# tjcunhao/dpo

Measured on NVIDIA H100. Metric: rtr_iters_per_sec_sphere2500, higher is better.
Workload: dtype f64

## Files before the change

### dpo_b200/csrc/dpgo_kernels.cu

```cuda
#include "dpgo_device.cuh"
#include "dpgo_kernels.cuh"
#include "dpgo_rotation.cuh"
#include <cooperative_groups.h>
#include <algorithm>

namespace dpgo {

struct BlockCtx {
  double *sm_warp;
  double *sm_out;
  unsigned epoch;
  int parity;
};

template <int NUSED = NRED>
__device__ __forceinline__ void phase_end(const KParams &kp, BlockCtx &bc, double (&acc)[NRED]) {
  const int lane = threadIdx.x & 31, warp = threadIdx.x >> 5, nwarps = blockDim.x >> 5;
#pragma unroll
  for (int q = 0; q < NUSED; ++q) {
    double v = warp_sum(acc[q]);
    if (lane == 0) bc.sm_warp[warp * NRED + q] = v;
  }
  __syncthreads();
  bc.epoch += gridDim.x;
  double *slot = kp.partials + (size_t)bc.parity * kp.grid * NRED;
  double *outp = bc.sm_out + bc.parity * NRED;
  if (warp == 0) {
    if (NUSED > 0) {
      double s[NUSED > 0 ? NUSED : 1];
#pragma unroll
      for (int q = 0; q < NUSED; ++q) {
        double v = (lane < nwarps) ? bc.sm_warp[lane * NRED + q] : 0.0;
        s[q] = warp_sum(v);
      }
      if (lane == 0) {
#pragma unroll
        for (int q = 0; q < NUSED; ++q) slot[(size_t)blockIdx.x * NRED + q] = s[q];
      }
    }
    if (!kp.cluster) {
      if (lane == 0) asm volatile("red.release.gpu.global.add.u32 [%0], 1;" ::"l"(kp.bar_counter) : "memory");
      if (kp.strict_acquire) { while ((int)(ld_acquire_u32(kp.bar_counter) - bc.epoch) < 0) { } }
      else { while ((int)(ld_relaxed_u32(kp.bar_counter) - bc.epoch) < 0) { } }
    }
  }
  if (kp.cluster) {
    asm volatile("barrier.cluster.arrive.release.aligned;" ::: "memory");
    if (kp.strict_acquire) asm volatile("barrier.cluster.wait.acquire.aligned;" ::: "memory");
    else asm volatile("barrier.cluster.wait.aligned;" ::: "memory");
  }
  if (warp == 0) {
    if (NUSED > 0) {
      double t[NUSED > 0 ? NUSED : 1];
#pragma unroll
      for (int q = 0; q < NUSED; ++q) t[q] = 0.0;
      for (int c = lane; c < kp.grid; c += 32) {
#pragma unroll
        for (int q = 0; q < NUSED; ++q) t[q] += __ldcg(slot + (size_t)c * NRED + q);
      }
#pragma unroll
      for (int q = 0; q < NUSED; ++q) {
        const double v = warp_sum(t[q]);
        if (lane == 0) outp[q] = v;
      }
    }
  }
  __syncthreads();
#pragma unroll
  for (int q = 0; q < NUSED; ++q) acc[q] = outp[q];
  bc.parity ^= 1;
}

struct CtaRows {
  int r0, r1;
  const int *rowptr;
  const int *bcol;
  const double *bval;
};

template <int R> struct RowIter {
  static constexpr int SG = SubGroup<R>::SG;
  int r0, r1, stride, jb, sgw, a, c;
  __device__ RowIter(const CtaRows &cr) {
    r0 = cr.r0;
    r1 = cr.r1;
    const int lane = threadIdx.x & 31;
    constexpr int SGW = 32 / SG;
    sgw = lane / SG;
    stride = (blockDim.x >> 5) * SGW;
    jb = r0 + (threadIdx.x >> 5) * SGW;
    const int l = lane & (SG - 1);
    a = l >> 2;
    c = l & 3;
  }
};

template <int R, int DH>
__device__ void phase_eval(const KParams &kp, const CtaRows &cr, int cb, bool save_xin, int precond, double (&acc)[NRED]) {
  constexpr int TS = R * DH;
  const double *X = kp.v[V_X0 + cb];
  double *EG = kp.v[V_EG0 + cb], *RG = kp.v[V_RG0 + cb], *Z0 = kp.v[V_Z00 + cb], *S = kp.S[cb];
  RowIter<R> it(cr);
  const bool valid = (it.a < R) && (it.c < DH);
  const int e = it.c * R + it.a;
  for (int jb = it.jb; jb < it.r1; jb += it.stride) {
    const int j = jb + it.sgw;
    const bool act = (j < it.r1);
    const int js = act ? j : it.r1 - 1;
    const bool ld = act && valid;
    double xq = gather_tile<R, DH, true, false>(cr.rowptr, cr.bcol, cr.bval, X, nullptr, 0.0, js, it.a, it.c);
    const size_t idx = (size_t)js * TS + e;
    const double x = ld ? __ldcg(X + idx) : 0.0;
    const double g = ld ? __ldcg(kp.G + idx) : 0.0;
    if (!ld) xq = 0.0;
    const double eg = xq + g;
    acc[0] = fma(xq, x, acc[0]);
    acc[1] = fma(x, g, acc[1]);
    double ya[3], sym[3];
    const double rg = tangent_project_elem<R, DH>(x, eg, it.a, it.c, ya, sym);
    if (ld) {
      EG[idx] = eg;
      RG[idx] = rg;
      if (save_xin) kp.v[V_XIN][idx] = x;
      acc[2] = fma(rg, rg, acc[2]);
    }
    if (act && it.a == 0 && it.c < 3) {
      double *s = S + (size_t)js * 9 + it.c * 3;
      s[0] = sym[0]; s[1] = sym[1]; s[2] = sym[2];
    }
    if (precond != DPGO_PRECOND_DENSE_EXACT && precond != DPGO_PRECOND_SPARSE_EXACT) {
      double z0 = rg;
      if (precond == DPGO_PRECOND_BLOCK_JACOBI) {
        double t = jacobi_elem<R, DH>(kp.dinv, js, ld ? rg : 0.0, it.a, it.c);
        double ya2[3], sym2[3];
        z0 = tangent_project_elem<R, DH>(x, t, it.a, it.c, ya2, sym2);
      }
      if (ld) {
        Z0[idx] = z0;
        acc[3] = fma(z0, rg, acc[3]);
      }
    }
  }
}

template <int R, int DH, bool CLOCK>
__device__ void phase_hess(const KParams &kp, const CtaRows &cr, int cb, const double *zsrc, const double *dold, double *dnew,
                           double beta, bool onfly, double (&acc)[NRED]) {
  constexpr int TS = R * DH;
  constexpr int D = DH - 1;
  const double *X = kp.v[V_X0 + cb];
  const double *S = kp.S[cb];
  double *HD = kp.v[V_HD];
  RowIter<R> it(cr);
  const bool valid = (it.a < R) && (it.c < DH);
  const int e = it.c * R + it.a;
  const bool ticking = CLOCK && (kp.phase_ns != nullptr) && blockIdx.x == 0 && threadIdx.x == 0;
  unsigned long long th0 = 0, th1 = 0;
  if (ticking) asm volatile("mov.u64 %0, %%globaltimer;" : "=l"(th0));
  for (int jb = it.jb; jb < it.r1; jb += it.stride) {
    const int j = jb + it.sgw;
    const bool act = (j < it.r1);
    const int js = act ? j : it.r1 - 1;
    const bool ld = act && valid;
    const size_t idx = (size_t)js * TS + e;
    double dl = 0.0, dprev = 0.0;
    if (ld) {
      dl = __ldcg(zsrc + idx);
      if (onfly && beta != 0.0) dprev = __ldcg(dold + idx);
    }
    const double x = ld ? __ldcg(X + idx) : 0.0;
    const bool rot = ld && (it.c < D);
    double s0 = 0, s1 = 0, s2 = 0;
    if (rot) {
      const double *s = S + (size_t)js * 9 + it.c * 3;
      s0 = __ldcg(s); s1 = __ldcg(s + 1); s2 = __ldcg(s + 2);
    }
    double hq;
    if (onfly) hq = gather_tile<R, DH, true, true>(cr.rowptr, cr.bcol, cr.bval, zsrc, dold, beta, js, it.a, it.c);
    else hq = gather_tile<R, DH, true, false>(cr.rowptr, cr.bcol, cr.bval, zsrc, nullptr, 0.0, js, it.a, it.c);
    if (ticking && jb == it.jb) { asm volatile("mov.u64 %0, %%globaltimer;" : "=l"(th1)); kp.phase_ns[27] += th1 - th0; }
    if (ld && onfly) {
      dl = -dl;
      if (beta != 0.0) dl = fma(beta, dprev, dl);
      dnew[idx] = dl;
    }
    const double dr = rot ? dl : 0.0;
    const double d0 = quad_get(dr, 0), d1 = quad_get(dr, 1), d2 = (D > 2) ? quad_get(dr, 2) : 0.0;
    double w = ld ? hq : 0.0;
    if (rot) w -= (d0 * s0 + d1 * s1 + d2 * s2);
    double ya[3], sym[3];
    const double hd = tangent_project_elem<R, DH>(x, w, it.a, it.c, ya, sym);
    if (ld) {
      HD[idx] = hd;
      acc[0] = fma(dl, hd, acc[0]);
    }
  }
  if (ticking) { asm volatile("mov.u64 %0, %%globaltimer;" : "=l"(th1)); kp.phase_ns[28] += th1 - th0; }
}

template <int R, int DH>
__device__ void phase_update(const KParams &kp, const CtaRows &cr, int cb, const double *dcur, double alpha, bool first, int precond,
                             double (&acc)[NRED]) {
  constexpr int TS = R * DH;
  const double *X = kp.v[V_X0 + cb];
  const double *RG = kp.v[V_RG0 + cb];
  double *ETA = kp.v[V_ETA], *RES = kp.v[V_RES], *Z = kp.v[V_Z];
  const double *HD = kp.v[V_HD];
  RowIter<R> it(cr);
  const bool valid = (it.a < R) && (it.c < DH);
  const int e = it.c * R + it.a;
  for (int jb = it.jb; jb < it.r1; jb += it.stride) {
    const int j = jb + it.sgw;
    const bool act = (j < it.r1);
    const int js = act ? j : it.r1 - 1;
    const bool ld = act && valid;
    const size_t idx = (size_t)js * TS + e;
    double res = 0.0, x = 0.0;
    if (ld) {
      const double dl = __ldcg(dcur + idx), hd = __ldcg(HD + idx);
      const double eta0 = first ? 0.0 : __ldcg(ETA + idx);
      const double res0 = first ? __ldcg(RG + idx) : __ldcg(RES + idx);
      res = fma(alpha, hd, res0);
      ETA[idx] = fma(alpha, dl, eta0);
      RES[idx] = res;
// ... 520 lines not shown
          }
        }
        d0 += f0;
        d1 += f1;
        {
          double *sl = slots + (size_t)slot * SLOT + r8 * R + 2 * k4;
          if (2 * k4 < R) sl[0] = accum ? sl[0] + d0 : d0;
          if (2 * k4 + 1 < R) sl[1] = accum ? sl[1] + d1 : d1;
        }
        ji = jn; ja = na; jb = nb;
      }
    }
    __syncthreads();
    if (ticking) asm volatile("mov.u64 %0, %%globaltimer;" : "=l"(tg2));
    {
      int eb = e0 + warp * SGW;
      int4 ea = make_int4(-1, 0, 0, 0), ec = make_int4(0, 0, 0, 0), ed = make_int4(0, 0, 0, 0);
      if (eb + sgw < e1) {
        const int4 *rp = reinterpret_cast<const int4 *>(N.epis + eb + sgw);
        ea = __ldg(rp); ec = __ldg(rp + 1); ed = __ldg(rp + 2);
      }
      while (eb < e1) {
        const int en = eb + nsub;
        int4 fa = make_int4(-1, 0, 0, 0), fc = make_int4(0, 0, 0, 0), fd = make_int4(0, 0, 0, 0);
        if (en + sgw < e1) {
          const int4 *rp = reinterpret_cast<const int4 *>(N.epis + en + sgw);
          fa = __ldg(rp); fc = __ldg(rp + 1); fd = __ldg(rp + 2);
        }
        const bool act = (eb + sgw < e1);
        const int kind = ea.x, slot0 = ea.y, nslots = ea.z, half = ea.w, out = ec.x, aux = ec.y, nc = ec.z, cext = ec.w;
        const bool ld = act && valid;
        const bool sol = (kind == nd::EPI_ROOT) || (kind == nd::EPI_B_OWN);
        double tval = 0.0, xq = 0.0, vv = 0.0, cv[NC] = {0.0, 0.0, 0.0, 0.0};
        if (ld) {
          if (kind == nd::EPI_B_OWN) tval = __ldcg(N.TX + (size_t)out * TS + e);
          if (sol) { xq = __ldcg(X + (size_t)aux * TS + e); vv = __ldcg(V + (size_t)aux * TS + e); }
          if (kind == nd::EPI_F_BND) {
            const int ci[NC] = {ed.x, ed.y, ed.z, ed.w};
#pragma unroll
            for (int q = 0; q < NC; ++q) cv[q] = (q < nc) ? __ldcg(N.C + (size_t)ci[q] * TS + e) : 0.0;
          }
        }
        double sum = 0.0;
        if (ld) {
          const double *sl = slots + (size_t)slot0 * SLOT + (half * DH + c) * R + a;
          for (int k = 0; k < nslots; ++k) sum += sl[(size_t)k * SLOT];
        }
        double x = 0.0;
        if (ld) {
          if (kind == nd::EPI_F_OWN) {
            N.TX[(size_t)out * TS + e] = sum;
          } else if (kind == nd::EPI_F_BND) {
#pragma unroll
            for (int q = 0; q < NC; ++q) sum += cv[q];
            for (int k = NC; k < nc; ++k) sum += __ldcg(N.C + (size_t)ld_const(N.csrc + cext + k - NC) * TS + e);
            N.C[(size_t)out * TS + e] = sum;
          } else if (sol) {
            x = (kind == nd::EPI_ROOT) ? sum : tval - sum;
            N.TX[(size_t)out * TS + e] = x;
          }
        }
        if (__any_sync(FULL, sol)) {
          double ya[3], sym[3];
          const double z = tangent_project_elem<R, DH>(sol ? xq : 0.0, x, a, c, ya, sym);
          if (ld && sol) {
            Zout[(size_t)aux * TS + e] = z;
            acc[0] = fma(z, vv, acc[0]);
          }
        }
        eb = en; ea = fa; ec = fc; ed = fd;
      }
    }
    if (ticking) {
      unsigned long long tg3;
      asm volatile("mov.u64 %0, %%globaltimer;" : "=l"(tg3));
      kp.phase_ns[24] += tg1 - tg0; kp.phase_ns[25] += tg2 - tg1; kp.phase_ns[26] += tg3 - tg2;
      unsigned long long *pp = kp.phase_ns + 32 + 3 * min(ph, 9);
      pp[0] += tg1 - tg0; pp[1] += tg2 - tg1; pp[2] += tg3 - tg2;
    }
    if (si + 1 < s1) __syncthreads();
  }
}

template <int R, int DH>
__device__ void phase_retract(const KParams &kp, const CtaRows &cr, int cb, int mode, const double *dcur, double tau, bool eta_zero,
                              double step, double (&acc)[NRED]) {
  constexpr int TS = R * DH;
  const double *X = kp.v[V_X0 + cb];
  const double *RG = kp.v[V_RG0 + cb];
  double *X2 = kp.v[V_X0 + (1 - cb)];
  RowIter<R> it(cr);
  const bool valid = (it.a < R) && (it.c < DH);
  const int e = it.c * R + it.a;
  for (int jb = it.jb; jb < it.r1; jb += it.stride) {
    const int j = jb + it.sgw;
    const bool act = (j < it.r1);
    const int js = act ? j : it.r1 - 1;
    const bool ld = act && valid;
    const size_t idx = (size_t)js * TS + e;
    double w = 0.0;
    if (ld) {
      const double x = __ldcg(X + idx);
      double eta;
      if (mode == 1) {
        eta = -step * __ldcg(RG + idx);
      } else if (mode == 2) {
        eta = __ldcg(kp.v[V_AUX] + idx);
      } else {
        const double g = __ldcg(RG + idx);
        eta = eta_zero ? 0.0 : __ldcg(kp.v[V_ETA] + idx);
        double heta = eta_zero ? 0.0 : (__ldcg(kp.v[V_RES] + idx) - g);
        if (tau != 0.0) {
          eta = fma(tau, __ldcg(dcur + idx), eta);
          heta = fma(tau, __ldcg(kp.v[V_HD] + idx), heta);
        }
        acc[0] = fma(eta, g, acc[0]);
        acc[1] = fma(eta, heta, acc[1]);
      }
      w = x + eta;
    }
    const double q = qf_retract_elem<R, DH>(w, it.a, it.c);
    if (ld) X2[idx] = q;
  }
}

template <int R, int DH> __device__ void phase_final(const KParams &kp, const CtaRows &cr, int cur, double (&acc)[NRED]) {
  constexpr int TS = R * DH;
  RowIter<R> it(cr);
  const bool valid = (it.a < R) && (it.c < DH);
  const int e = it.c * R + it.a;
  for (int jb = it.jb; jb < it.r1; jb += it.stride) {
    const int j = jb + it.sgw;
    if (j < it.r1 && valid) {
      const size_t idx = (size_t)j * TS + e;
      const double x = __ldcg(kp.v[V_X0 + cur] + idx);
      const double d = x - __ldcg(kp.v[V_XIN] + idx);
      acc[0] = fma(d, d, acc[0]);
      if (cur != 0) kp.v[V_X0][idx] = x;
    }
  }
}

__device__ __forceinline__ void zero(double (&acc)[NRED]) {
#pragma unroll
  for (int q = 0; q < NRED; ++q) acc[q] = 0.0;
}

template <int R, int DH, bool FULL> __global__ void __launch_bounds__(OPT_THREADS, 1) k_optimize(const KParams kp) {
  if (kp.gate != nullptr && __ldg(kp.gate) == 0) return;
  extern __shared__ double smem[];
  BlockCtx bc;
  bc.sm_warp = smem;
  bc.sm_out = smem + (OPT_THREADS / 32) * NRED;
  int *sp_ints = reinterpret_cast<int *>(bc.sm_out + 2 * NRED);
  CtaRows cr;
  cr.r0 = ld_const(kp.cta_rows + blockIdx.x);
  cr.r1 = ld_const(kp.cta_rows + blockIdx.x + 1);
  cr.rowptr = kp.rowptr;
  cr.bcol = kp.bcol;
  cr.bval = kp.bval;
  {
    const int nrows = cr.r1 - cr.r0;
    const int blk0 = (nrows > 0) ? ld_const(kp.rowptr + cr.r0) : 0, blk1 = (nrows > 0) ? ld_const(kp.rowptr + cr.r1) : 0;
    if (nrows > 0 && nrows + 1 + (blk1 - blk0) <= SP_CACHE_INTS) {
      for (int q = threadIdx.x; q <= nrows; q += blockDim.x) sp_ints[q] = ld_const(kp.rowptr + cr.r0 + q) - blk0;
      for (int q = threadIdx.x; q < blk1 - blk0; q += blockDim.x) sp_ints[nrows + 1 + q] = ld_const(kp.bcol + blk0 + q);
      cr.rowptr = sp_ints - cr.r0;
      cr.bcol = sp_ints + nrows + 1;
      cr.bval = kp.bval + (size_t)blk0 * 16;
    }
    __syncthreads();
  }
  double *sV = reinterpret_cast<double *>(sp_ints + SP_CACHE_INTS);
  DenseRing ring;
  ring.buf = sV + (size_t)DENSE_PER_MAX * R;
  ring.full = reinterpret_cast<uint64_t *>(ring.buf + (size_t)DENSE_RING_DOUBLES);
  ring.empty = ring.full + DENSE_NST;
  ring.count = 0;
  int *sMeta = reinterpret_cast<int *>(ring.empty + DENSE_NST);
  const bool dense_tma = FULL && (kp.prm.precond == DPGO_PRECOND_DENSE_EXACT) && (kp.pinv != nullptr) && ((kp.N & 1) == 0) &&
                         (kp.N >= 2048);
  const bool dense_sym = dense_tma && (kp.sym_ok != 0);
  if (dense_tma) {
    if (dense_sym) {
      for (int q = threadIdx.x; q < DENSE_RING_DOUBLES; q += blockDim.x) ring.buf[q] = 0.0;
    }
    if (threadIdx.x == 0) {
      for (int st = 0; st < DENSE_NST; ++st) {
        asm volatile("mbarrier.init.shared::cta.b64 [%0], %1;" ::"r"(smem_addr(&ring.full[st])), "r"(1));
        asm volatile("mbarrier.init.shared::cta.b64 [%0], %1;" ::"r"(smem_addr(&ring.empty[st])), "r"(OPT_THREADS / 32 - 1));
      }
      asm volatile("fence.mbarrier_init.release.cluster;" ::: "memory");
    }
    __syncthreads();
  }
  bc.epoch = *kp.bar_epoch;
  bc.parity = 0;
  unsigned long long tick_last = 0;
  const bool ticking = FULL && (kp.phase_ns != nullptr) && blockIdx.x == 0 && threadIdx.x == 0;
  auto tick = [&](int kind) {
    if (ticking) {
      unsigned long long t;
      asm volatile("mov.u64 %0, %%globaltimer;" : "=l"(t));
      if (kind >= 0) kp.phase_ns[kind] += t - tick_last;
      tick_last = t;
    }
  };
  tick(-1);
  const dpgo_opt_params_t prm = kp.prm;
  const int precond = prm.precond;
  const bool exact = (precond == DPGO_PRECOND_DENSE_EXACT) || (precond == DPGO_PRECOND_SPARSE_EXACT);
  dpgo_opt_result_t res;
  res.success = 0; res.tcg_status = DPGO_TCG_NOT_RUN; res.tcg_iterations = 0; res.outer_iterations = 0;
  res.rejections = 0; res.spmv_passes = 0; res.precond_applies = 0; res.reserved0 = 0;
  res.f_init = res.gradnorm_init = res.f_opt = res.gradnorm_opt = res.relative_change = res.elapsed_ms = 0.0;
  res.quad_init = res.lin_init = 0.0;
  double acc[NRED];
  double *nd_ys = sV;
  double *nd_slots = sV + (size_t)kp.nd.max_ytiles * R * DH;
  int4 *nd_grec = reinterpret_cast<int4 *>((reinterpret_cast<uintptr_t>(nd_slots + (size_t)kp.nd.max_slots * nd::PANEL_ROWS * R) + 15) & ~(uintptr_t)15);
  double *nd_res = reinterpret_cast<double *>(nd_grec + 2 * (size_t)kp.nd.max_gathers);
  auto apply_exact = [&](const double *Vv, int cbx, double *Zout) {
    if (!FULL || precond == DPGO_PRECOND_SPARSE_EXACT) {
      zero(acc);
      for (int ph = 0; ph < kp.nd.nphases; ++ph) {
        phase_nd<R, DH, FULL>(kp, ph, Vv, cbx, Zout, nd_ys, nd_slots, nd_grec, nd_res, res.precond_applies == 0, acc);
        if (ph + 1 < kp.nd.nphases) { phase_end<0>(kp, bc, acc); tick(8 + min(ph, 15)); }
      }
      phase_end<1>(kp, bc, acc);
      tick(8 + min(kp.nd.nphases - 1, 15));
    } else {
      if (dense_sym) phase_dense_sym<R>(kp, Vv, ring, sV, sMeta);
      else if (dense_tma) phase_dense_tma<R>(kp, Vv, sV, ring);
      else phase_dense<R>(kp, Vv, sV);
      zero(acc); phase_end<0>(kp, bc, acc);
      tick(1);
      zero(acc); phase_pz<R, DH>(kp, cr, cbx, Vv, Zout, sV, acc);
      phase_end<1>(kp, bc, acc);
      tick(2);
    }
  };

  int cur = 0;

  if (kp.op == OP_PHASE_BENCH) {
    for (int i = 0; i < prm.tr_max_inner; ++i) { zero(acc); acc[0] = 1.0; phase_end<1>(kp, bc, acc); }
    if (blockIdx.x == 0 && threadIdx.x == 0) { res.f_init = acc[0]; *kp.result = res; *kp.bar_epoch = bc.epoch; }
    return;
  }
  if (kp.op == OP_PRECON) {
    if (exact) {
      apply_exact(kp.v[V_AUX], 0, kp.v[V_Z]);
    } else {
      constexpr int TS = R * DH;
      RowIter<R> it(cr);
      const bool valid = (it.a < R) && (it.c < DH);
      const int e = it.c * R + it.a;
      for (int jb = it.jb; jb < it.r1; jb += it.stride) {
        const int j = jb + it.sgw;
        const bool act = (j < it.r1);
        const int js = act ? j : it.r1 - 1;
        const bool ld = act && valid;
        const size_t idx = (size_t)js * TS + e;
        const double x = ld ? __ldcg(kp.v[V_X0] + idx) : 0.0;
        double t = ld ? __ldcg(kp.v[V_AUX] + idx) : 0.0;
        if (precond == DPGO_PRECOND_BLOCK_JACOBI) t = jacobi_elem<R, DH>(kp.dinv, js, t, it.a, it.c);
        double ya[3], sym[3];
        const double z = tangent_project_elem<R, DH>(x, t, it.a, it.c, ya, sym);
        if (ld) kp.v[V_Z][idx] = z;
      }
      zero(acc); phase_end(kp, bc, acc);
    }
    if (blockIdx.x == 0 && threadIdx.x == 0) *kp.bar_epoch = bc.epoch;
    return;
  }
  if (kp.op == OP_RETRACT) {
    zero(acc);
    phase_retract<R, DH>(kp, cr, 0, 2, nullptr, 0.0, false, 0.0, acc);
    phase_end(kp, bc, acc);
    if (blockIdx.x == 0 && threadIdx.x == 0) *kp.bar_epoch = bc.epoch;
    return;
  }

  zero(acc);
  phase_eval<R, DH>(kp, cr, 0, true, precond, acc);
  phase_end(kp, bc, acc);
  tick(0);
  res.spmv_passes++;
  double f1 = 0.5 * acc[0] + acc[1];
  double gn = sqrt(acc[2]);
  double zr0 = acc[3];
  res.f_init = f1;
  res.gradnorm_init = gn;
  res.quad_init = acc[0];
  res.lin_init = acc[1];
  res.f_opt = f1;
  res.gradnorm_opt = gn;

  if (kp.op == OP_EVAL) {
    res.success = 1;
    if (blockIdx.x == 0 && threadIdx.x == 0) { *kp.result = res; *kp.bar_epoch = bc.epoch; }
    return;
  }
  if (kp.op == OP_RHESS) {
    zero(acc);
    phase_hess<R, DH, FULL>(kp, cr, 0, kp.v[V_AUX], nullptr, nullptr, 0.0, false, acc);
    phase_end(kp, bc, acc);
    if (blockIdx.x == 0 && threadIdx.x == 0) { *kp.result = res; *kp.bar_epoch = bc.epoch; }
    return;
  }

  if (prm.algorithm == DPGO_ALG_RGD) {
    zero(acc);
    phase_retract<R, DH>(kp, cr, 0, 1, nullptr, 0.0, false, prm.rgd_stepsize, acc);
    phase_end(kp, bc, acc);
    zero(acc);
    phase_eval<R, DH>(kp, cr, 1, false, DPGO_PRECOND_NONE, acc);
    phase_end(kp, bc, acc);
    res.spmv_passes++;
    res.f_opt = 0.5 * acc[0] + acc[1];
    res.gradnorm_opt = sqrt(acc[2]);
    res.outer_iterations = 1;
    cur = 1;
  } else if (gn >= prm.tr_tolerance) {
    const bool single = (prm.tr_iterations == 1);
    double Delta = prm.tr_initial_radius;
    const double Delta_max = single ? Delta : 5.0 * prm.tr_initial_radius;
    int total_steps = 0;
    int cb = 0;
    bool z0_valid = !exact;
    int iter = 0;
    while (true) {
      if (!z0_valid) {
        apply_exact(kp.v[V_RG0 + cb], cb, kp.v[V_Z00 + cb]);
        zr0 = acc[0];
        z0_valid = true;
      }
      double z_r = zr0, d_Pd = zr0, e_Pd = 0.0, e_Pe = 0.0;
      const double n0 = gn;
      res.precond_applies++;
      double beta = 0.0, tau = 0.0;
      const double *zsrc = kp.v[V_Z00 + cb];
      int pd = 0;
      bool eta_zero = true;
      int status = DPGO_TCG_MAXITER;
      const double *dcur = nullptr;
      for (int j = 0; j < prm.tr_max_inner; ++j) {
        double *dnew = kp.v[V_D0 + (1 - pd)];
        zero(acc);
        phase_hess<R, DH, FULL>(kp, cr, cb, zsrc, kp.v[V_D0 + pd], dnew, beta, true, acc);
        phase_end<1>(kp, bc, acc);
        tick(3);
        res.spmv_passes++;
        res.tcg_iterations++;
        pd = 1 - pd;
        dcur = dnew;
        const double d_Hd = acc[0];
        const double alpha = z_r / d_Hd;
        const double e_new = e_Pe + 2.0 * alpha * e_Pd + alpha * alpha * d_Pd;
        if (d_Hd <= 0.0 || e_new >= Delta * Delta) {
          tau = (-e_Pd + sqrt(e_Pd * e_Pd + d_Pd * (Delta * Delta - e_Pe))) / d_Pd;
          status = (d_Hd <= 0.0) ? DPGO_TCG_NEGCURVTURE : DPGO_TCG_EXCREGION;
          break;
        }
        e_Pe = e_new;
        zero(acc);
        phase_update<R, DH>(kp, cr, cb, dcur, alpha, eta_zero, precond, acc);
        phase_end<2>(kp, bc, acc);
        tick(4);
        eta_zero = false;
        const double nr = sqrt(acc[0]);
        const double n0t = n0;
        if (nr <= n0 * fmin(n0t, 0.1)) {
          status = (0.1 < n0t) ? DPGO_TCG_LCON : DPGO_TCG_SCON;
          break;
        }
        double zr_new = acc[1];
        if (exact) {
          apply_exact(kp.v[V_RES], cb, kp.v[V_Z]);
          zr_new = acc[0];
        }
        res.precond_applies++;
        beta = zr_new / z_r;
        z_r = zr_new;
        zsrc = kp.v[V_Z];
        e_Pd = beta * (e_Pd + alpha * d_Pd);
        d_Pd = z_r + beta * beta * d_Pd;
      }
      res.tcg_status = status;
      res.outer_iterations++;
      zero(acc);
      phase_retract<R, DH>(kp, cr, cb, 0, dcur, tau, eta_zero, 0.0, acc);
      phase_end<2>(kp, bc, acc);
      tick(5);
      const double denom = -acc[0] - 0.5 * acc[1];
      zero(acc);
      phase_eval<R, DH>(kp, cr, 1 - cb, false, precond, acc);
      phase_end(kp, bc, acc);
      tick(0);
      res.spmv_passes++;
      const double f2 = 0.5 * acc[0] + acc[1];
      const double gn2 = sqrt(acc[2]);
      const double rho = (denom != 0.0) ? (f1 - f2) / denom : -1.0;
      const bool accepted = rho > 0.1;
      if (single) {
        if (accepted) {
          cb = 1 - cb; res.f_opt = f2; res.gradnorm_opt = gn2;
          break;
        }
        res.rejections++;
        if (total_steps > 10) break;
        Delta *= 0.25;
        total_steps++;
      } else {
        if (rho < 0.25) Delta *= 0.25;
        else if (rho > 0.75 && (status == DPGO_TCG_NEGCURVTURE || status == DPGO_TCG_EXCREGION))
          Delta = fmin(2.0 * Delta, Delta_max);
        if (accepted) {
          cb = 1 - cb; f1 = f2; gn = gn2; zr0 = acc[3];
          res.f_opt = f2; res.gradnorm_opt = gn2;
          z0_valid = !exact;
        } else {
          res.rejections++;
        }
        ++iter;
        if (gn < prm.tr_tolerance || iter >= prm.tr_iterations) break;
      }
    }
    cur = cb;
  }

  zero(acc);
  phase_final<R, DH>(kp, cr, cur, acc);
  phase_end<1>(kp, bc, acc);
  tick(6);
  res.relative_change = sqrt(acc[0] / (double)kp.n);
  res.success = 1;
  if (blockIdx.x == 0 && threadIdx.x == 0) {
    *kp.result = res;
    *kp.bar_epoch = bc.epoch;
    if (kp.opt_record) { kp.opt_record[0] = res.relative_change; kp.opt_record[1] += 1.0; }
  }
}

constexpr int SPMV_THREADS = 256;

template <int R, int DH>
__global__ void __launch_bounds__(SPMV_THREADS) k_spmv(int n, const int *__restrict__ rowptr,
                                                       const int *__restrict__ bcol,
                                                       const double *__restrict__ bval,
                                                       const double *__restrict__ X,
                                                       const double *__restrict__ G, double *__restrict__ out) {
  constexpr int SG = SubGroup<R>::SG;
  constexpr int TS = R * DH;
  const int lane = threadIdx.x & 31;
  const int l = lane & (SG - 1), a = l >> 2, c = l & 3;
  const int sg_global = (blockIdx.x * SPMV_THREADS + threadIdx.x) / SG;
  const int j = sg_global;
  const bool act = j < n;
  const int js = act ? j : n - 1;
  double v = gather_tile<R, DH, false, false>(rowptr, bcol, bval, X, nullptr, 0.0, js, a, c);
  if (act && a < R && c < DH) {
    const size_t idx = (size_t)js * TS + c * R + a;
    if (G != nullptr) v += __ldg(G + idx);
    out[idx] = v;
  }
}

template <int R, int DH> __global__ void k_stiefel_project(int n, const double *M, double *out, double c0, const double *B, double c1,
                                                            const double *Cc, double c2) {
  constexpr int TS = R * DH;
  const int j = blockIdx.x * blockDim.x + threadIdx.x;
  if (j >= n) return;
  stiefel_project_tile<R, DH>(
      [&](int e) {
        double v = c0 * M[(size_t)j * TS + e];
        if (B) v = fma(c1, B[(size_t)j * TS + e], v);
        if (Cc) v = fma(c2, Cc[(size_t)j * TS + e], v);
        return v;
      },
      [&](int e, double v) { out[(size_t)j * TS + e] = v; });
}

__global__ void k_pack_tiles(int ts, int count, const int *__restrict__ pose, const double *__restrict__ X,
                             double *__restrict__ out, const unsigned char *__restrict__ gate) {
  const int t = blockIdx.x * blockDim.x + threadIdx.x;
  if (t >= count * ts || (gate != nullptr && *gate == 0)) return;
  const int s = t / ts, e = t - s * ts;
  out[t] = X[(size_t)pose[s] * ts + e];
}

template <int R, int DH>
__global__ void k_build_G(int nposes, const int *__restrict__ pose_ids, const int *__restrict__ pose_ptr,
                          const int *__restrict__ edge_slot, const int *__restrict__ edge_out,
                          const double *__restrict__ edge_T, const double *__restrict__ edge_om,
                          const double *__restrict__ gathered, double *__restrict__ G,
                          const unsigned char *__restrict__ gate) {
  constexpr int TS = R * DH;
  const int t = blockIdx.x * blockDim.x + threadIdx.x;
  if (t >= nposes * TS || (gate != nullptr && *gate == 0)) return;
  const int pi = t / TS, e = t - pi * TS;
  const int c = e / R, a = e - c * R;
  double acc = 0.0;
  for (int k = pose_ptr[pi]; k < pose_ptr[pi + 1]; ++k) {
    const double *Xn = gathered + (size_t)edge_slot[k] * TS;
    const double *T = edge_T + (size_t)k * DH * DH;
    const double *om = edge_om + (size_t)k * DH;
    double s = 0.0;
    if (edge_out[k]) {
#pragma unroll
      for (int q = 0; q < DH; ++q) s = fma(Xn[q * R + a] * om[q], T[c * DH + q], s);
    } else {
#pragma unroll
      for (int q = 0; q < DH; ++q) s = fma(Xn[q * R + a], T[q * DH + c], s);
      s *= om[c];
    }
    acc -= s;
  }
  G[(size_t)pose_ids[pi] * TS + e] = acc;
}

__global__ void k_assemble_Q(int64_t nb, const int *__restrict__ cptr, const int2 *__restrict__ contrib, const double *__restrict__ eT,
                             const double *__restrict__ eom, const double *__restrict__ ew, const double *__restrict__ sblk,
                             double *__restrict__ bval) {
  const int64_t tid = (int64_t)blockIdx.x * blockDim.x + threadIdx.x;
  if (tid >= nb * 16) return;
  const int64_t b = tid >> 4;
  const int k = (int)((tid >> 2) & 3), c = (int)(tid & 3);
  double v = 0.0;
  for (int q = cptr[b]; q < cptr[b + 1]; ++q) {
    const int2 cc = contrib[q];
    if (cc.y == 4) { v += sblk[(size_t)cc.x * 16 + k * 4 + c]; continue; }
    const double *T = eT + (size_t)cc.x * 16, *om = eom + (size_t)cc.x * 4;
    const double w = ew[cc.x];
    if (cc.y == 0) {
      double s = 0.0;
#pragma unroll
      for (int u = 0; u < 4; ++u) s = fma(T[k * 4 + u] * (om[u] * w), T[c * 4 + u], s);
      v += s;
    } else if (cc.y == 1) {
      if (k == c) v += om[k] * w;
    } else if (cc.y == 2) {
      v -= T[k * 4 + c] * (om[c] * w);
    } else {
      v -= (om[k] * w) * T[c * 4 + k];
    }
  }
  bval[tid] = v;
}

template <int R, int DH>
__global__ void k_edge_weights(int64_t m, const int *__restrict__ p1, const int *__restrict__ p2, const double *__restrict__ eT,
                               const double *__restrict__ eom, const int *__restrict__ fixed, const double *__restrict__ X, int cost,
                               double mu, double param, double *__restrict__ w, double *__restrict__ resid,
                               unsigned long long *__restrict__ gnc) {
  constexpr int D = DH - 1, TS = R * DH;
  const int64_t e = (int64_t)blockIdx.x * blockDim.x + threadIdx.x;
  if (e >= m) return;
  const double *T = eT + (size_t)e * 16, *om = eom + (size_t)e * 4;
  const double *X1 = X + (size_t)p1[e] * TS, *X2 = X + (size_t)p2[e] * TS;
  double rot = 0.0, tra = 0.0;
  for (int a = 0; a < R; ++a) {
    for (int c = 0; c < D; ++c) {
      double s = -X2[c * R + a];
      for (int q = 0; q < D; ++q) s = fma(X1[q * R + a], T[q * 4 + c], s);
      rot = fma(s, s, rot);
    }
    double s = X2[D * R + a] - X1[D * R + a];
    for (int q = 0; q < D; ++q) s = fma(-X1[q * R + a], T[q * 4 + D], s);
    tra = fma(s, s, tra);
  }
  const double r2 = om[0] * rot + om[D] * tra;
  if (resid) resid[e] = r2;
  if (fixed && fixed[e]) return;
  const double r = sqrt(r2);
  double wt = 1.0;
  if (cost == 1) wt = 1.0 / r;
  else if (cost == 2) wt = (r < param) ? 1.0 : param / r;
  else if (cost == 3) wt = (r < param) ? 1.0 : 0.0;
  else if (cost == 4) { const double s = 1.0 + r2; wt = 1.0 / (s * s); }
  else if (cost == 5) wt = gnc_tls_weight(r2, mu, param);
  w[e] = wt;
  if (gnc) atomicAdd(gnc + (wt == 1.0 ? 0 : (wt == 0.0 ? 1 : 2)), 1ULL);
}

template <int R, int DH> static size_t nd_staged_doubles(const KNd &nd) {
  return (OPT_THREADS / 32) * NRED + 2 * NRED + SP_CACHE_INTS / 2 + (size_t)nd.max_ytiles * R * DH +
         (size_t)(nd.max_slots + 1) * nd::PANEL_ROWS * R + 4 * (size_t)nd.max_gathers + 8;
}

template <int R, int DH> static size_t optimize_smem_doubles(const KParams &kp) {
  const size_t base = (OPT_THREADS / 32) * NRED + 2 * NRED + SP_CACHE_INTS / 2;
  const size_t dense = (size_t)DENSE_PER_MAX * R + (size_t)DENSE_RING_DOUBLES + 2 * DENSE_NST + (size_t)SYM_META_DOUBLES;
  if (kp.prm.precond == DPGO_PRECOND_DENSE_EXACT) return base + dense;
  if (kp.prm.precond == DPGO_PRECOND_SPARSE_EXACT) return nd_staged_doubles<R, DH>(kp.nd) + (size_t)kp.nd.resident_doubles;
  return base + 8;
}

int64_t nd_resident_budget(int r, int dh, const KNd &nd) {
  int64_t staged = 0;
  DPGO_DISPATCH(r, dh, staged = (int64_t)nd_staged_doubles<R, DH>(nd) * (int64_t)sizeof(double));
  return std::max<int64_t>(0, (int64_t)OPT_SMEM_LIMIT - staged);
}

template <int R, int DH> static void *optimize_kernel(bool full) {
  return full ? (void *)k_optimize<R, DH, true> : (void *)k_optimize<R, DH, false>;
}

template <int R, int DH> static cudaError_t launch_optimize_t(const KParams &kp_in, cudaStream_t stream) {
  KParams kp = kp_in;
  const bool full = (kp.phase_ns != nullptr) || (kp.prm.precond == DPGO_PRECOND_DENSE_EXACT);
  const void *kern = optimize_kernel<R, DH>(full);
  static_assert((size_t)ND_YCAP_TILES * R * DH + (size_t)(ND_SLOT_CAP + 1) * nd::PANEL_ROWS * R + 4 * (size_t)ND_YCAP_TILES + 8 <=
                    (size_t)DENSE_PER_MAX * R + (size_t)DENSE_RING_DOUBLES + 2 * DENSE_NST + (size_t)SYM_META_DOUBLES,
                "the sparse plan's capacities must fit the kernel's maximum shared memory");
  kp.smem_doubles = (int)optimize_smem_doubles<R, DH>(kp);
  const size_t smem = (size_t)kp.smem_doubles * sizeof(double);
  static bool attr_set[2][64] = {};
  int dev = 0;
  cudaGetDevice(&dev);
  if (dev < 0 || dev >= 64 || !attr_set[full][dev]) {
    cudaError_t e = cudaFuncSetAttribute(kern, cudaFuncAttributeMaxDynamicSharedMemorySize, OPT_SMEM_LIMIT);
    if (e != cudaSuccess) return e;
    if (dev >= 0 && dev < 64) attr_set[full][dev] = true;
  }
  {
    static int last_pct[2][64];
    static bool init = false;
    if (!init) { for (int i = 0; i < 64; ++i) last_pct[0][i] = last_pct[1][i] = -1; init = true; }
    const int pct = std::min(100, (int)((smem + 2048) * 100 / (228 * 1024)) + 1);
    if (dev >= 0 && dev < 64 && last_pct[full][dev] != pct) {
      cudaFuncSetAttribute(kern, cudaFuncAttributePreferredSharedMemoryCarveout, pct);
      last_pct[full][dev] = pct;
    }
  }
  if (kp.cluster) {
    static bool np_set[2][64] = {};
    if (kp.grid > 8 && (dev < 0 || dev >= 64 || !np_set[full][dev])) {
      cudaError_t e = cudaFuncSetAttribute(kern, cudaFuncAttributeNonPortableClusterSizeAllowed, 1);
      if (e != cudaSuccess) return e;
      if (dev >= 0 && dev < 64) np_set[full][dev] = true;
    }
    cudaLaunchConfig_t cfg = {};
    cfg.gridDim = dim3(kp.grid);
    cfg.blockDim = dim3(OPT_THREADS);
    cfg.dynamicSmemBytes = smem;
    cfg.stream = stream;
    cudaLaunchAttribute at[1];
    at[0].id = cudaLaunchAttributeClusterDimension;
    at[0].val.clusterDim.x = (unsigned)kp.grid;
    at[0].val.clusterDim.y = 1;
    at[0].val.clusterDim.z = 1;
    cfg.attrs = at;
    cfg.numAttrs = 1;
    void *args[] = {(void *)&kp};
    return cudaLaunchKernelExC(&cfg, kern, args);
  }
  void *args[] = {(void *)&kp};
  return cudaLaunchCooperativeKernel(kern, dim3(kp.grid), dim3(OPT_THREADS), args, smem, stream);
}

template <int R, int DH> static int max_cluster_t(int device) {
  const size_t smem = OPT_SMEM_LIMIT;
  for (int f = 0; f < 2; ++f) {
    cudaFuncSetAttribute(optimize_kernel<R, DH>(f != 0), cudaFuncAttributeNonPortableClusterSizeAllowed, 1);
    cudaFuncSetAttribute(optimize_kernel<R, DH>(f != 0), cudaFuncAttributeMaxDynamicSharedMemorySize, OPT_SMEM_LIMIT);
  }
  for (int cs : {16, 8}) {
    cudaLaunchConfig_t cfg = {};
    cfg.gridDim = dim3(cs);
    cfg.blockDim = dim3(OPT_THREADS);
    cfg.dynamicSmemBytes = smem;
    cudaLaunchAttribute at[1];
    at[0].id = cudaLaunchAttributeClusterDimension;
    at[0].val.clusterDim.x = (unsigned)cs;
    at[0].val.clusterDim.y = 1;
    at[0].val.clusterDim.z = 1;
    cfg.attrs = at;
    cfg.numAttrs = 1;
    int n0 = 0, n1 = 0;
    if (cudaOccupancyMaxActiveClusters(&n0, optimize_kernel<R, DH>(false), &cfg) == cudaSuccess && n0 >= 1 &&
        cudaOccupancyMaxActiveClusters(&n1, optimize_kernel<R, DH>(true), &cfg) == cudaSuccess && n1 >= 1)
      return cs;
  }
  cudaGetLastError();
  return 0;
}

template <int R, int DH> static int max_grid_t(int device) {
  const size_t smem = OPT_SMEM_LIMIT;
  int per_sm = 1, sms = 0, optin = 0;
  if (cudaDeviceGetAttribute(&optin, cudaDevAttrMaxSharedMemoryPerBlockOptin, device) != cudaSuccess || optin < OPT_SMEM_LIMIT)
    return 0;
  for (int f = 0; f < 2; ++f) {
    const void *kern = optimize_kernel<R, DH>(f != 0);
    cudaFuncSetAttribute(kern, cudaFuncAttributeMaxDynamicSharedMemorySize, (int)smem);
    int ps = 0;
    if (cudaOccupancyMaxActiveBlocksPerMultiprocessor(&ps, kern, OPT_THREADS, smem) != cudaSuccess) return 0;
    per_sm = std::min(per_sm, ps);
  }
  if (cudaDeviceGetAttribute(&sms, cudaDevAttrMultiProcessorCount, device) != cudaSuccess) return 0;
  return per_sm > 0 ? sms : 0;
}

cudaError_t launch_optimize(int r, int dh, const KParams &kp, cudaStream_t stream) {
  cudaError_t e = cudaErrorInvalidValue;
  DPGO_DISPATCH(r, dh, e = (launch_optimize_t<R, DH>(kp, stream)));
  return e;
}

int optimize_max_grid(int r, int dh, int device) {
  int g = 0;
  DPGO_DISPATCH(r, dh, g = (max_grid_t<R, DH>(device)));
  return g;
}

int optimize_max_cluster(int r, int dh, int device) {
  int g = 0;
  DPGO_DISPATCH(r, dh, g = (max_cluster_t<R, DH>(device)));
  return g;
}

cudaError_t launch_spmv(int r, int dh, int n, const int *rowptr, const int *bcol, const double *bval,
                        const double *X, const double *G, double *out, cudaStream_t stream) {
  bool ok = false;
  DPGO_DISPATCH(r, dh, {
    constexpr int SG = SubGroup<R>::SG;
    const int per_block = SPMV_THREADS / SG;
    const int blocks = (n + per_block - 1) / per_block;
    k_spmv<R, DH><<<blocks, SPMV_THREADS, 0, stream>>>(n, rowptr, bcol, bval, X, G, out);
    ok = true;
  });
  if (!ok) return cudaErrorInvalidValue;
  return cudaGetLastError();
}

cudaError_t launch_stiefel_project(int r, int dh, int n, const double *M, double *out, cudaStream_t stream, double c0,
                                   const double *B, double c1, const double *C, double c2) {
  bool ok = false;
  DPGO_DISPATCH(r, dh, {
    k_stiefel_project<R, DH><<<(n + 127) / 128, 128, 0, stream>>>(n, M, out, c0, B, c1, C, c2);
    ok = true;
  });
  if (!ok) return cudaErrorInvalidValue;
  return cudaGetLastError();
// ... 99 lines not shown
```

Baseline: 2043.

## Move trust-region scalar solver state into shared memory updated by one lane

The scalar trust-region and truncated-CG bookkeeping (alpha, beta, Delta, result counters, break flags) moves out of per-thread registers into a shared-memory SolverState. Lane 0 of warp 0 updates it through a callback inside phase_end, before the block-wide sync. This is meant to cut register pressure and the redundant scalar math every thread did after each grid reduction. The cost is extra shared-memory reads of state on the critical path and a larger static shared footprint, which shrinks what is left for the sparse-row cache.

Result: faster. 2241, median of 6 (+9.7%).

```diff
diff --git a/dpo_b200/csrc/dpgo_kernels.cu b/dpo_b200/csrc/dpgo_kernels.cu
--- a/dpo_b200/csrc/dpgo_kernels.cu
+++ b/dpo_b200/csrc/dpgo_kernels.cu
@@ -13,8 +13,12 @@
   int parity;
 };
 
-template <int NUSED = NRED>
-__device__ __forceinline__ void phase_end(const KParams &kp, BlockCtx &bc, double (&acc)[NRED]) {
+struct NoUpdate {
+  __device__ void operator()(const double *) const {}
+};
+
+template <int NUSED = NRED, class Update = NoUpdate>
+__device__ __forceinline__ void phase_end(const KParams &kp, BlockCtx &bc, double (&acc)[NRED], const Update &update = Update()) {
   const int lane = threadIdx.x & 31, warp = threadIdx.x >> 5, nwarps = blockDim.x >> 5;
 #pragma unroll
   for (int q = 0; q < NUSED; ++q) {
@@ -64,12 +68,28 @@
         if (lane == 0) outp[q] = v;
       }
     }
+    if (lane == 0) update(outp);
   }
   __syncthreads();
 #pragma unroll
   for (int q = 0; q < NUSED; ++q) acc[q] = outp[q];
   bc.parity ^= 1;
 }
+
+struct SolverState {
+  dpgo_opt_result_t res;
+  double f1, gn, zr0;
+  double Delta, Delta_max;
+  double z_r, d_Pd, e_Pd, e_Pe, n0, alpha, beta, tau;
+  double denom;
+  int cb;
+  int pd;
+  int zsrc_z;
+  int eta_zero, z0_valid, status, iter, total_steps;
+  int brk;
+  unsigned long long tick_last;
+};
+constexpr int STATE_DOUBLES = (int)((sizeof(SolverState) + 15) / 16) * 2;
 
 struct CtaRows {
   int r0, r1;
@@ -896,7 +916,15 @@
   BlockCtx bc;
   bc.sm_warp = smem;
   bc.sm_out = smem + (OPT_THREADS / 32) * NRED;
-  int *sp_ints = reinterpret_cast<int *>(bc.sm_out + 2 * NRED);
+  SolverState &S = *reinterpret_cast<SolverState *>(bc.sm_out + 2 * NRED);
+  if (threadIdx.x == 0) {
+    dpgo_opt_result_t &res = S.res;
+    res.success = 0; res.tcg_status = DPGO_TCG_NOT_RUN; res.tcg_iterations = 0; res.outer_iterations = 0;
+    res.rejections = 0; res.spmv_passes = 0; res.precond_applies = 0; res.reserved0 = 0;
+    res.f_init = res.gradnorm_init = res.f_opt = res.gradnorm_opt = res.relative_change = res.elapsed_ms = 0.0;
+    res.quad_init = res.lin_init = 0.0;
+  }
+  int *sp_ints = reinterpret_cast<int *>(bc.sm_out + 2 * NRED + STATE_DOUBLES);
   CtaRows cr;
   cr.r0 = ld_const(kp.cta_rows + blockIdx.x);
   cr.r1 = ld_const(kp.cta_rows + blockIdx.x + 1);
@@ -940,38 +968,30 @@
   }
   bc.epoch = *kp.bar_epoch;
   bc.parity = 0;
-  unsigned long long tick_last = 0;
-  const bool ticking = FULL && (kp.phase_ns != nullptr) && blockIdx.x == 0 && threadIdx.x == 0;
   auto tick = [&](int kind) {
-    if (ticking) {
+    if (FULL && kp.phase_ns != nullptr && blockIdx.x == 0 && threadIdx.x == 0) {
       unsigned long long t;
       asm volatile("mov.u64 %0, %%globaltimer;" : "=l"(t));
-      if (kind >= 0) kp.phase_ns[kind] += t - tick_last;
-      tick_last = t;
+      if (kind >= 0) kp.phase_ns[kind] += t - S.tick_last;
+      S.tick_last = t;
     }
   };
   tick(-1);
-  const dpgo_opt_params_t prm = kp.prm;
-  const int precond = prm.precond;
+  const int precond = kp.prm.precond;
   const bool exact = (precond == DPGO_PRECOND_DENSE_EXACT) || (precond == DPGO_PRECOND_SPARSE_EXACT);
-  dpgo_opt_result_t res;
-  res.success = 0; res.tcg_status = DPGO_TCG_NOT_RUN; res.tcg_iterations = 0; res.outer_iterations = 0;
-  res.rejections = 0; res.spmv_passes = 0; res.precond_applies = 0; res.reserved0 = 0;
-  res.f_init = res.gradnorm_init = res.f_opt = res.gradnorm_opt = res.relative_change = res.elapsed_ms = 0.0;
-  res.quad_init = res.lin_init = 0.0;
   double acc[NRED];
   double *nd_ys = sV;
   double *nd_slots = sV + (size_t)kp.nd.max_ytiles * R * DH;
   int4 *nd_grec = reinterpret_cast<int4 *>((reinterpret_cast<uintptr_t>(nd_slots + (size_t)kp.nd.max_slots * nd::PANEL_ROWS * R) + 15) & ~(uintptr_t)15);
   double *nd_res = reinterpret_cast<double *>(nd_grec + 2 * (size_t)kp.nd.max_gathers);
-  auto apply_exact = [&](const double *Vv, int cbx, double *Zout) {
+  auto apply_exact = [&](const double *Vv, int cbx, double *Zout, const auto &update) {
     if (!FULL || precond == DPGO_PRECOND_SPARSE_EXACT) {
       zero(acc);
       for (int ph = 0; ph < kp.nd.nphases; ++ph) {
-        phase_nd<R, DH, FULL>(kp, ph, Vv, cbx, Zout, nd_ys, nd_slots, nd_grec, nd_res, res.precond_applies == 0, acc);
+        phase_nd<R, DH, FULL>(kp, ph, Vv, cbx, Zout, nd_ys, nd_slots, nd_grec, nd_res, S.res.precond_applies == 0, acc);
         if (ph + 1 < kp.nd.nphases) { phase_end<0>(kp, bc, acc); tick(8 + min(ph, 15)); }
       }
-      phase_end<1>(kp, bc, acc);
+      phase_end<1>(kp, bc, acc, update);
       tick(8 + min(kp.nd.nphases - 1, 15));
     } else {
       if (dense_sym) phase_dense_sym<R>(kp, Vv, ring, sV, sMeta);
@@ -980,7 +1000,7 @@
       zero(acc); phase_end<0>(kp, bc, acc);
       tick(1);
       zero(acc); phase_pz<R, DH>(kp, cr, cbx, Vv, Zout, sV, acc);
-      phase_end<1>(kp, bc, acc);
+      phase_end<1>(kp, bc, acc, update);
       tick(2);
     }
   };
@@ -988,13 +1008,13 @@
   int cur = 0;
 
   if (kp.op == OP_PHASE_BENCH) {
-    for (int i = 0; i < prm.tr_max_inner; ++i) { zero(acc); acc[0] = 1.0; phase_end<1>(kp, bc, acc); }
-    if (blockIdx.x == 0 && threadIdx.x == 0) { res.f_init = acc[0]; *kp.result = res; *kp.bar_epoch = bc.epoch; }
+    for (int i = 0; i < kp.prm.tr_max_inner; ++i) { zero(acc); acc[0] = 1.0; phase_end<1>(kp, bc, acc); }
+    if (blockIdx.x == 0 && threadIdx.x == 0) { S.res.f_init = acc[0]; *kp.result = S.res; *kp.bar_epoch = bc.epoch; }
     return;
   }
   if (kp.op == OP_PRECON) {
     if (exact) {
-      apply_exact(kp.v[V_AUX], 0, kp.v[V_Z]);
+      apply_exact(kp.v[V_AUX], 0, kp.v[V_Z], NoUpdate());
     } else {
       constexpr int TS = R * DH;
       RowIter<R> it(cr);
@@ -1026,164 +1046,185 @@
     return;
   }
 
+  const bool single = (kp.prm.tr_iterations == 1);
+  auto tcg_begin = [&]() {
+    S.z_r = S.zr0; S.d_Pd = S.zr0; S.e_Pd = 0.0; S.e_Pe = 0.0;
+    S.n0 = S.gn;
+    S.res.precond_applies++;
+    S.beta = 0.0; S.tau = 0.0;
+    S.zsrc_z = 0; S.pd = 0; S.eta_zero = 1; S.status = DPGO_TCG_MAXITER;
+  };
+  auto tcg_next = [&](double zr_new) {
+    S.res.precond_applies++;
+    const double beta = zr_new / S.z_r;
+    S.beta = beta;
+    S.z_r = zr_new;
+    S.zsrc_z = 1;
+    S.e_Pd = beta * (S.e_Pd + S.alpha * S.d_Pd);
+    S.d_Pd = S.z_r + beta * beta * S.d_Pd;
+  };
   zero(acc);
   phase_eval<R, DH>(kp, cr, 0, true, precond, acc);
-  phase_end(kp, bc, acc);
+  phase_end(kp, bc, acc, [&](const double *t) {
+    dpgo_opt_result_t &res = S.res;
+    res.spmv_passes++;
+    const double f1 = 0.5 * t[0] + t[1];
+    const double gn = sqrt(t[2]);
+    S.f1 = f1; S.gn = gn; S.zr0 = t[3];
+    res.f_init = f1;
+    res.gradnorm_init = gn;
+    res.quad_init = t[0];
+    res.lin_init = t[1];
+    res.f_opt = f1;
+    res.gradnorm_opt = gn;
+    S.Delta = kp.prm.tr_initial_radius;
+    S.Delta_max = single ? S.Delta : 5.0 * kp.prm.tr_initial_radius;
+    S.total_steps = 0; S.cb = 0; S.iter = 0;
+    S.z0_valid = !exact;
+    if (kp.op != OP_EVAL && kp.op != OP_RHESS && kp.prm.algorithm != DPGO_ALG_RGD && gn >= kp.prm.tr_tolerance && !exact)
+      tcg_begin();
+  });
   tick(0);
-  res.spmv_passes++;
-  double f1 = 0.5 * acc[0] + acc[1];
-  double gn = sqrt(acc[2]);
-  double zr0 = acc[3];
-  res.f_init = f1;
-  res.gradnorm_init = gn;
-  res.quad_init = acc[0];
-  res.lin_init = acc[1];
-  res.f_opt = f1;
-  res.gradnorm_opt = gn;
 
   if (kp.op == OP_EVAL) {
-    res.success = 1;
-    if (blockIdx.x == 0 && threadIdx.x == 0) { *kp.result = res; *kp.bar_epoch = bc.epoch; }
+    if (blockIdx.x == 0 && threadIdx.x == 0) { S.res.success = 1; *kp.result = S.res; *kp.bar_epoch = bc.epoch; }
     return;
   }
   if (kp.op == OP_RHESS) {
     zero(acc);
     phase_hess<R, DH, FULL>(kp, cr, 0, kp.v[V_AUX], nullptr, nullptr, 0.0, false, acc);
     phase_end(kp, bc, acc);
-    if (blockIdx.x == 0 && threadIdx.x == 0) { *kp.result = res; *kp.bar_epoch = bc.epoch; }
+    if (blockIdx.x == 0 && threadIdx.x == 0) { *kp.result = S.res; *kp.bar_epoch = bc.epoch; }
     return;
   }
 
-  if (prm.algorithm == DPGO_ALG_RGD) {
+  if (kp.prm.algorithm == DPGO_ALG_RGD) {
     zero(acc);
-    phase_retract<R, DH>(kp, cr, 0, 1, nullptr, 0.0, false, prm.rgd_stepsize, acc);
+    phase_retract<R, DH>(kp, cr, 0, 1, nullptr, 0.0, false, kp.prm.rgd_stepsize, acc);
     phase_end(kp, bc, acc);
     zero(acc);
     phase_eval<R, DH>(kp, cr, 1, false, DPGO_PRECOND_NONE, acc);
-    phase_end(kp, bc, acc);
-    res.spmv_passes++;
-    res.f_opt = 0.5 * acc[0] + acc[1];
-    res.gradnorm_opt = sqrt(acc[2]);
-    res.outer_iterations = 1;
+    phase_end(kp, bc, acc, [&](const double *t) {
+      S.res.spmv_passes++;
+      S.res.f_opt = 0.5 * t[0] + t[1];
+      S.res.gradnorm_opt = sqrt(t[2]);
+      S.res.outer_iterations = 1;
+    });
     cur = 1;
-  } else if (gn >= prm.tr_tolerance) {
-    const bool single = (prm.tr_iterations == 1);
-    double Delta = prm.tr_initial_radius;
-    const double Delta_max = single ? Delta : 5.0 * prm.tr_initial_radius;
-    int total_steps = 0;
-    int cb = 0;
-    bool z0_valid = !exact;
-    int iter = 0;
+  } else if (S.gn >= kp.prm.tr_tolerance) {
     while (true) {
-      if (!z0_valid) {
-        apply_exact(kp.v[V_RG0 + cb], cb, kp.v[V_Z00 + cb]);
-        zr0 = acc[0];
-        z0_valid = true;
-      }
-      double z_r = zr0, d_Pd = zr0, e_Pd = 0.0, e_Pe = 0.0;
-      const double n0 = gn;
-      res.precond_applies++;
-      double beta = 0.0, tau = 0.0;
-      const double *zsrc = kp.v[V_Z00 + cb];
-      int pd = 0;
-      bool eta_zero = true;
-      int status = DPGO_TCG_MAXITER;
-      const double *dcur = nullptr;
-      for (int j = 0; j < prm.tr_max_inner; ++j) {
-        double *dnew = kp.v[V_D0 + (1 - pd)];
+      if (!S.z0_valid) {
+        const int cb = S.cb;
+        apply_exact(kp.v[V_RG0 + cb], cb, kp.v[V_Z00 + cb], [&](const double *t) {
+          S.zr0 = t[0];
+          S.z0_valid = 1;
+          tcg_begin();
+        });
+      }
+      for (int j = 0; j < kp.prm.tr_max_inner; ++j) {
+        {
+          const int cb = S.cb, pd = S.pd;
+          zero(acc);
+          phase_hess<R, DH, FULL>(kp, cr, cb, S.zsrc_z ? kp.v[V_Z] : kp.v[V_Z00 + cb], kp.v[V_D0 + pd], kp.v[V_D0 + (1 - pd)],
+                                  S.beta, true, acc);
+        }
+        phase_end<1>(kp, bc, acc, [&](const double *t) {
+          S.res.spmv_passes++;
+          S.res.tcg_iterations++;
+          S.pd = 1 - S.pd;
+          const double d_Hd = t[0];
+          const double Delta = S.Delta, e_Pd = S.e_Pd, d_Pd = S.d_Pd, e_Pe = S.e_Pe;
+          const double alpha = S.z_r / d_Hd;
+          const double e_new = e_Pe + 2.0 * alpha * e_Pd + alpha * alpha * d_Pd;
+          S.alpha = alpha;
+          S.brk = d_Hd <= 0.0 || e_new >= Delta * Delta;
+          if (S.brk) {
+            S.tau = (-e_Pd + sqrt(e_Pd * e_Pd + d_Pd * (Delta * Delta - e_Pe))) / d_Pd;
+            S.status = (d_Hd <= 0.0) ? DPGO_TCG_NEGCURVTURE : DPGO_TCG_EXCREGION;
+          } else {
+            S.e_Pe = e_new;
+          }
+        });
+        tick(3);
+        if (S.brk) break;
         zero(acc);
-        phase_hess<R, DH, FULL>(kp, cr, cb, zsrc, kp.v[V_D0 + pd], dnew, beta, true, acc);
-        phase_end<1>(kp, bc, acc);
-        tick(3);
+        phase_update<R, DH>(kp, cr, S.cb, kp.v[V_D0 + S.pd], S.alpha, S.eta_zero, precond, acc);
+        phase_end<2>(kp, bc, acc, [&](const double *t) {
+          S.eta_zero = 0;
+          const double nr = sqrt(t[0]);
+          const double n0 = S.n0;
+          const double n0t = n0;
+          S.brk = nr <= n0 * fmin(n0t, 0.1);
+          if (S.brk) S.status = (0.1 < n0t) ? DPGO_TCG_LCON : DPGO_TCG_SCON;
+          else if (!exact) tcg_next(t[1]);
+        });
+        tick(4);
+        if (S.brk) break;
+        if (exact) apply_exact(kp.v[V_RES], S.cb, kp.v[V_Z], [&](const double *t) { tcg_next(t[0]); });
+      }
+      zero(acc);
+      phase_retract<R, DH>(kp, cr, S.cb, 0, kp.v[V_D0 + S.pd], S.tau, S.eta_zero, 0.0, acc);
+      phase_end<2>(kp, bc, acc, [&](const double *t) {
+        S.res.tcg_status = S.status;
+        S.res.outer_iterations++;
+        S.denom = -t[0] - 0.5 * t[1];
+      });
+      tick(5);
+      zero(acc);
+      phase_eval<R, DH>(kp, cr, 1 - S.cb, false, precond, acc);
+      phase_end(kp, bc, acc, [&](const double *t) {
+        dpgo_opt_result_t &res = S.res;
         res.spmv_passes++;
-        res.tcg_iterations++;
-        pd = 1 - pd;
-        dcur = dnew;
-        const double d_Hd = acc[0];
-        const double alpha = z_r / d_Hd;
-        const double e_new = e_Pe + 2.0 * alpha * e_Pd + alpha * alpha * d_Pd;
-        if (d_Hd <= 0.0 || e_new >= Delta * Delta) {
-          tau = (-e_Pd + sqrt(e_Pd * e_Pd + d_Pd * (Delta * Delta - e_Pe))) / d_Pd;
-          status = (d_Hd <= 0.0) ? DPGO_TCG_NEGCURVTURE : DPGO_TCG_EXCREGION;
-          break;
-        }
-        e_Pe = e_new;
-        zero(acc);
-        phase_update<R, DH>(kp, cr, cb, dcur, alpha, eta_zero, precond, acc);
-        phase_end<2>(kp, bc, acc);
-        tick(4);
-        eta_zero = false;
-        const double nr = sqrt(acc[0]);
-        const double n0t = n0;
-        if (nr <= n0 * fmin(n0t, 0.1)) {
-          status = (0.1 < n0t) ? DPGO_TCG_LCON : DPGO_TCG_SCON;
-          break;
-        }
-        double zr_new = acc[1];
-        if (exact) {
-          apply_exact(kp.v[V_RES], cb, kp.v[V_Z]);
-          zr_new = acc[0];
-        }
-        res.precond_applies++;
-        beta = zr_new / z_r;
-        z_r = zr_new;
-        zsrc = kp.v[V_Z];
-        e_Pd = beta * (e_Pd + alpha * d_Pd);
-        d_Pd = z_r + beta * beta * d_Pd;
-      }
-      res.tcg_status = status;
-      res.outer_iterations++;
-      zero(acc);
-      phase_retract<R, DH>(kp, cr, cb, 0, dcur, tau, eta_zero, 0.0, acc);
-      phase_end<2>(kp, bc, acc);
-      tick(5);
-      const double denom = -acc[0] - 0.5 * acc[1];
-      zero(acc);
-      phase_eval<R, DH>(kp, cr, 1 - cb, false, precond, acc);
-      phase_end(kp, bc, acc);
+        const double f2 = 0.5 * t[0] + t[1];
+        const double gn2 = sqrt(t[2]);
+        const double denom = S.denom;
+        const double rho = (denom != 0.0) ? (S.f1 - f2) / denom : -1.0;
+        const bool accepted = rho > 0.1;
+        if (single) {
+          if (accepted) {
+            S.cb = 1 - S.cb; res.f_opt = f2; res.gradnorm_opt = gn2;
+            S.brk = 1;
+          } else {
+            res.rejections++;
+            S.brk = S.total_steps > 10;
+            if (!S.brk) {
+              S.Delta *= 0.25;
+              S.total_steps++;
+            }
+          }
+        } else {
+          if (rho < 0.25) S.Delta *= 0.25;
+          else if (rho > 0.75 && (S.status == DPGO_TCG_NEGCURVTURE || S.status == DPGO_TCG_EXCREGION))
+            S.Delta = fmin(2.0 * S.Delta, S.Delta_max);
+          if (accepted) {
+            S.cb = 1 - S.cb; S.f1 = f2; S.gn = gn2; S.zr0 = t[3];
+            res.f_opt = f2; res.gradnorm_opt = gn2;
+            S.z0_valid = !exact;
+          } else {
+            res.rejections++;
+          }
+          ++S.iter;
+          S.brk = S.gn < kp.prm.tr_tolerance || S.iter >= kp.prm.tr_iterations;
+        }
+        if (!S.brk && S.z0_valid) tcg_begin();
+      });
       tick(0);
-      res.spmv_passes++;
-      const double f2 = 0.5 * acc[0] + acc[1];
-      const double gn2 = sqrt(acc[2]);
-      const double rho = (denom != 0.0) ? (f1 - f2) / denom : -1.0;
-      const bool accepted = rho > 0.1;
-      if (single) {
-        if (accepted) {
-          cb = 1 - cb; res.f_opt = f2; res.gradnorm_opt = gn2;
-          break;
-        }
-        res.rejections++;
-        if (total_steps > 10) break;
-        Delta *= 0.25;
-        total_steps++;
-      } else {
-        if (rho < 0.25) Delta *= 0.25;
-        else if (rho > 0.75 && (status == DPGO_TCG_NEGCURVTURE || status == DPGO_TCG_EXCREGION))
-          Delta = fmin(2.0 * Delta, Delta_max);
-        if (accepted) {
-          cb = 1 - cb; f1 = f2; gn = gn2; zr0 = acc[3];
-          res.f_opt = f2; res.gradnorm_opt = gn2;
-          z0_valid = !exact;
-        } else {
-          res.rejections++;
-        }
-        ++iter;
-        if (gn < prm.tr_tolerance || iter >= prm.tr_iterations) break;
-      }
-    }
-    cur = cb;
+      if (S.brk) break;
+    }
+    cur = S.cb;
   }
 
   zero(acc);
   phase_final<R, DH>(kp, cr, cur, acc);
-  phase_end<1>(kp, bc, acc);
+  phase_end<1>(kp, bc, acc, [&](const double *t) {
+    S.res.relative_change = sqrt(t[0] / (double)kp.n);
+    S.res.success = 1;
+  });
   tick(6);
-  res.relative_change = sqrt(acc[0] / (double)kp.n);
-  res.success = 1;
   if (blockIdx.x == 0 && threadIdx.x == 0) {
-    *kp.result = res;
+    *kp.result = S.res;
     *kp.bar_epoch = bc.epoch;
-    if (kp.opt_record) { kp.opt_record[0] = res.relative_change; kp.opt_record[1] += 1.0; }
+    if (kp.opt_record) { kp.opt_record[0] = S.res.relative_change; kp.opt_record[1] += 1.0; }
   }
 }
 
@@ -1328,13 +1369,15 @@
   if (gnc) atomicAdd(gnc + (wt == 1.0 ? 0 : (wt == 0.0 ? 1 : 2)), 1ULL);
 }
 
+constexpr size_t OPT_SMEM_BASE_DOUBLES = (OPT_THREADS / 32) * NRED + 2 * NRED + STATE_DOUBLES + SP_CACHE_INTS / 2;
+
 template <int R, int DH> static size_t nd_staged_doubles(const KNd &nd) {
-  return (OPT_THREADS / 32) * NRED + 2 * NRED + SP_CACHE_INTS / 2 + (size_t)nd.max_ytiles * R * DH +
-         (size_t)(nd.max_slots + 1) * nd::PANEL_ROWS * R + 4 * (size_t)nd.max_gathers + 8;
+  return OPT_SMEM_BASE_DOUBLES + (size_t)nd.max_ytiles * R * DH + (size_t)(nd.max_slots + 1) * nd::PANEL_ROWS * R +
+         4 * (size_t)nd.max_gathers + 8;
 }
 
 template <int R, int DH> static size_t optimize_smem_doubles(const KParams &kp) {
-  const size_t base = (OPT_THREADS / 32) * NRED + 2 * NRED + SP_CACHE_INTS / 2;
+  const size_t base = OPT_SMEM_BASE_DOUBLES;
   const size_t dense = (size_t)DENSE_PER_MAX * R + (size_t)DENSE_RING_DOUBLES + 2 * DENSE_NST + (size_t)SYM_META_DOUBLES;
   if (kp.prm.precond == DPGO_PRECOND_DENSE_EXACT) return base + dense;
   if (kp.prm.precond == DPGO_PRECOND_SPARSE_EXACT) return nd_staged_doubles<R, DH>(kp.nd) + (size_t)kp.nd.resident_doubles;
```
